# pyprob/pyprob

Hardware: NVIDIA H100
Metric: ic_train_traces_per_sec (higher is better)
Workload: dtype f32

## Files before the change

pyprob_b200/csrc/obs_embed.inc:

```

struct ObsLayout {
  int in_off[PPB_MAX_OBS], out_off[PPB_MAX_OBS];
  int max_depth;
};
inline ObsLayout obs_layout(const ppb_net_desc& D) {
  ObsLayout o;
  int ci = 0, co = 0;
  o.max_depth = 0;
  for (int j = 0; j < D.num_obs; ++j) {
    o.in_off[j] = ci; o.out_off[j] = co;
    ci += D.obs_ff[j].in_dim; co += D.obs_ff[j].out_dim;
    o.max_depth = D.obs_ff[j].num_layers > o.max_depth ? D.obs_ff[j].num_layers : o.max_depth;
  }
  return o;
}

template <class W>
void obs_fp32_plan_fwd(Builder& bl, const ppb_net_desc& D, const float* arena, const float* obs, int B, const W& w,
                       float* obs_emb) {
  const int E = D.obs_dim;
  const ObsLayout o = obs_layout(D);
  for (int l = 0; l < o.max_depth; ++l) {
    bl.begin();
    for (int j = 0; j < D.num_obs; ++j) {
// ... 92 lines not shown

inline obsmlp::Plan obs_plan_of(const ppb_net_desc& D, const Ws* w, const float* obs) {
  obsmlp::Plan P;
  memset(&P, 0, sizeof(P));
  const int E = D.obs_dim;
  const ObsLayout lay = obs_layout(D);
  P.E = E;
  int nf = 0;
  auto add_layer = [&](const ppb_linear_desc& L) -> obsmlp::Layer& {
    obsmlp::Layer& o = P.L[P.n_layers++];
    o.in_dim = L.in_dim; o.out_dim = L.out_dim; o.w_off = L.w_off; o.b_off = L.b_off;
    o.pitch = (L.in_dim & 3) ? L.in_dim : ((L.in_dim & 7) ? L.in_dim : L.in_dim + 4);
    o.sw = nf;
    nf += (L.out_dim * o.pitch + L.out_dim + 3) & ~3;
    o.part = P.part_floats;
    P.part_floats += L.out_dim * L.in_dim + L.out_dim;
    return o;
  };
  std::vector<int> first(D.num_obs);
  for (int j = 0; j < D.num_obs; ++j) {
    const ppb_ff_desc& ff = D.obs_ff[j];
    first[j] = P.n_layers;
    for (int l = 0; l < ff.num_layers; ++l) {
      obsmlp::Layer& o = add_layer(ff.layers[l]);
      o.xoff = P.A; P.A += o.in_dim;
      if (l + 1 < ff.num_layers) { o.dzoff = P.Dz; P.Dz += o.out_dim; }
      o.dxoff = l == 0 ? -1 : P.L[P.n_layers - 2].dzoff;
      o.x = l == 0 ? obs + lay.in_off[j] : (w ? w->obs_act[j][l - 1] : nullptr);
      o.ldx = l == 0 ? D.obs_in_total : ff.layers[l - 1].out_dim;
      if (l + 1 < ff.num_layers) { o.y = w ? w->obs_act[j][l] : nullptr; o.ldy = o.out_dim; }
    }
  }
  const int cat = P.A, dcat = P.Dz;
  P.A += E; P.Dz += E;
  for (int j = 0; j < D.num_obs; ++j) {
    obsmlp::Layer& o = P.L[first[j] + D.obs_ff[j].num_layers - 1];
    o.yoff = cat + lay.out_off[j]; o.dzoff = dcat + lay.out_off[j];
    o.y = w ? w->obs_cat + lay.out_off[j] : nullptr; o.ldy = E;
  }
  for (int j = 0; j < D.num_obs; ++j)
    for (int l = 0; l + 1 < D.obs_ff[j].num_layers; ++l) P.L[first[j] + l].yoff = P.L[first[j] + l + 1].xoff;
  const int nfin = D.obs_final.num_layers;
  for (int l = 0; l < nfin; ++l) {
    const bool last = l == nfin - 1;
    obsmlp::Layer& o = add_layer(D.obs_final.layers[l]);
    if (l == 0) o.xoff = cat;
    o.yoff = P.A; P.A += o.out_dim;
    o.dzoff = P.Dz; P.Dz += o.out_dim;
    o.dxoff = l == 0 ? dcat : P.L[P.n_layers - 2].dzoff;
    o.x = l == 0 ? (w ? w->obs_cat : nullptr) : (w ? w->fin_act[l - 1] : nullptr);
    o.ldx = o.in_dim;
    o.y = w ? (last ? w->obs_emb : w->fin_act[l]) : nullptr; o.ldy = o.out_dim;
    if (l > 0) o.xoff = P.L[P.n_layers - 2].yoff;
  }
  P.w_floats = nf;
  return P;
}
inline bool obs_fused_ok(const ppb_net_desc& D) {
  constexpr int kFuseMaxWidth = obsmlp::W2;
  if (D.obs_dim > kFuseMaxWidth) return false;
  for (int j = 0; j < D.num_obs; ++j)
    for (int l = 0; l < D.obs_ff[j].num_layers; ++l)
      if (D.obs_ff[j].layers[l].in_dim > kFuseMaxWidth || D.obs_ff[j].layers[l].out_dim > kFuseMaxWidth) return false;
  for (int l = 0; l < D.obs_final.num_layers; ++l)
    if (D.obs_final.layers[l].in_dim > kFuseMaxWidth || D.obs_final.layers[l].out_dim > kFuseMaxWidth) return false;
  const obsmlp::Plan P = obs_plan_of(D, nullptr, nullptr);
  return obsmlp::smem_fwd(P) <= obsmlp::kMaxSmem && obsmlp::smem_bwd(P) <= obsmlp::kMaxSmem;
}
int obs_fused_fwd(const ppb_net_desc& D, const float* arena, const float* obs, int B, const Ws& w, cudaStream_t st,
                  const HImg* emb_img = nullptr) {
  int rc = smem_opt_in<obsmlp::k_fwd>(obsmlp::kMaxSmem);
  if (rc) return rc;
  obsmlp::Plan P = obs_plan_of(D, &w, obs);
  if (emb_img) {
    P.emb_k_hi = emb_img->k_hi; P.emb_k_lo = emb_img->k_lo; P.emb_mn_hi = emb_img->mn_hi; P.emb_mn_lo = emb_img->mn_lo;
    P.emb_kb = emb_img->kb;
  }
  const int tpc = (B + PPB_NUM_SMS - 1) / PPB_NUM_SMS;
  PPB_CUDA(ppb_launch(obsmlp::k_fwd, dim3((B + tpc - 1) / tpc), dim3(obsmlp::kThreads), obsmlp::smem_fwd(P), st, 1, 0, P, arena,
                      B, tpc));
  PPB_LAUNCH_CHECK();
  return PPB_OK;
}
int obs_fused_bwd(const ppb_net_desc& D, const float* arena, float* grad, const float* obs, int B, const Ws& w,
                  cudaStream_t st) {
  int rc = smem_opt_in<obsmlp::k_bwd>(obsmlp::kMaxSmem);
  if (rc) return rc;
  const obsmlp::Plan P = obs_plan_of(D, &w, obs);
  constexpr int kMaxCtas = 16 * obsmlp::kCluster;
  int tpc = (B + kMaxCtas - 1) / kMaxCtas;
  tpc = tpc < obsmlp::kMT ? obsmlp::kMT : tpc;
  int ctas = (B + tpc - 1) / tpc;
  ctas = (ctas + obsmlp::kCluster - 1) / obsmlp::kCluster * obsmlp::kCluster;
  PPB_CUDA(ppb_launch(obsmlp::k_bwd, dim3(ctas), dim3(obsmlp::kThreads), obsmlp::smem_bwd(P), st, 1, obsmlp::kCluster, P, arena,
                      (const float*)w.d_obs_emb, grad, B, tpc));
  PPB_LAUNCH_CHECK();
  return PPB_OK;
}

inline bool obs_tc_ok(const ppb_net_desc& D) {
  const ObsLayout o = obs_layout(D);
  for (int j = 0; j < D.num_obs; ++j) {
    const ppb_ff_desc& ff = D.obs_ff[j];
    if (ff.num_layers < 2 || (o.out_off[j] & 31)) return false;
    for (int l = 1; l < ff.num_layers; ++l)
      if (ff.layers[l].in_dim < 32) return false;
  }
  for (int l = 0; l < D.obs_final.num_layers; ++l)
    if (D.obs_final.layers[l].in_dim < 32) return false;
  return true;
}

template <class Add>
void obs_weight_images(ppb_net* net, Add add) {
  const ppb_net_desc& D = net->desc;
  net->obs_form = obs_fused_ok(D) ? ObsForm::fused : obs_tc_ok(D) ? ObsForm::tensor_core : ObsForm::simt;
  if (net->obs_form != ObsForm::tensor_core) return;
  for (int j = 0; j < D.num_obs; ++j)
    for (int l = 1; l < D.obs_ff[j].num_layers; ++l) {
      const ppb_linear_desc& L = D.obs_ff[j].layers[l];
      net->w_obs[j][l] = add(L.w_off, L.out_dim, L.in_dim, L.in_dim);
    }
  for (int l = 0; l < D.obs_final.num_layers; ++l) {
    const ppb_linear_desc& L = D.obs_final.layers[l];
    net->w_fin[l] = add(L.w_off, L.out_dim, L.in_dim, L.in_dim);
  }
}

struct ObsImgs {
  HImg act[PPB_MAX_OBS][PPB_MAX_FF_LAYERS], cat, fin[PPB_MAX_FF_LAYERS];
  HImg g_act[PPB_MAX_OBS][PPB_MAX_FF_LAYERS], g_cat, g_fin[PPB_MAX_FF_LAYERS], g_emb;
  char* begin; int64_t bytes;
};
template <class Img>
void obs_carve_images(const ppb_net* net, int B, Img img, ObsImgs& o) {
  if (net->obs_form != ObsForm::tensor_core) return;
  const ppb_net_desc& D = net->desc;
  for (int j = 0; j < D.num_obs; ++j)
    for (int l = 0; l + 1 < D.obs_ff[j].num_layers; ++l) {
      o.act[j][l] = img(B, D.obs_ff[j].layers[l].out_dim);
      o.g_act[j][l] = img(B, D.obs_ff[j].layers[l].out_dim);
    }
  o.cat = img(B, D.obs_dim);
  o.g_cat = img(B, D.obs_dim);
  for (int l = 0; l + 1 < D.obs_final.num_layers; ++l) {
    o.fin[l] = img(B, D.obs_final.layers[l].out_dim);
    o.g_fin[l] = img(B, D.obs_final.layers[l].out_dim);
  }
  o.g_emb = img(B, D.obs_dim);
}

__global__ void __launch_bounds__(256) k_pack_rows_masked(float* __restrict__ g, const float* __restrict__ y, int rows,
                                                           int cols, int64_t ld, HImg img) {
  ppb_pdl_trigger();
  ppb_pdl_wait();
  tc::pack_tile<tc::Parts::both>(blockIdx.x, (int)img.kb, img.k_hi, img.k_lo, img.mn_hi, img.mn_lo,
                                 [&](int row, int k0, float (&x)[4]) {
#pragma unroll
    for (int j = 0; j < 4; ++j) {
      x[j] = 0.0f;
      if (row < rows && k0 + j < cols) {
        const int64_t o = (int64_t)row * ld + k0 + j;
        x[j] = y[o] > 0.0f ? g[o] : 0.0f;
        g[o] = x[j];
      }
    }
  });
}

struct ObsStep {
  Builder bl;
  std::vector<int> tc_ph;
  int tc_dw = -1;
};

int obs_plan_fwd(ppb_net* net, const float* arena, const ppb_batch* b, const Ws& w, const ObsImgs& im, const HImg& emb_img,
                 TcBuilder& tb, ObsStep& os, cudaStream_t st) {
  const ppb_net_desc& D = net->desc;
// ... 57 lines not shown
  if (net->obs_form != ObsForm::tensor_core) {
    if (!emb_packed) {
      PPB_CUDA(ppb_launch(k_pack_rows, dim3(dim3((B + 127) / 128, 4)), dim3(256), 0, st, 1, 0, w.obs_emb, B, E, E, emb_img));
      PPB_LAUNCH_CHECK();
    }
    return stream_after(net, s_img, st);
  }
  for (int j = 0; j < D.num_obs; ++j) {
    const int od = D.obs_ff[j].layers[0].out_dim;
    PPB_CUDA(ppb_launch(k_pack_rows, dim3(dim3((B + 127) / 128, 4)), dim3(256), 0, st, 1, 0, w.obs_act[j][0], B, od, od, im.act[j][0]));
    PPB_LAUNCH_CHECK();
  }
  rc = stream_after(net, s_img, st); if (rc) return rc;
  for (int ph : os.tc_ph) { rc = run_tc_phase_auto<2>(tb.phases[ph], tdev, precision, st, tb); if (rc) return rc; }
  return PPB_OK;
}

int obs_plan_bwd(ppb_net* net, const float* arena, float* grad, const ppb_batch* b, const Ws& w, const ObsImgs& im,
                 TcBuilder& tb, ObsStep& os, cudaStream_t st) {
  const ppb_net_desc& D = net->desc;
  const int B = b->n_traces;
  const ObsLayout o = obs_layout(D);
  if (net->obs_form == ObsForm::simt) obs_fp32_plan_bwd(os.bl, D, arena, grad, b->obs, B, w);
  if (net->obs_form == ObsForm::tensor_core) {
    os.bl.begin();
    for (int j = 0; j < D.num_obs; ++j) {
      const ppb_linear_desc& L = D.obs_ff[j].layers[0];
      os.bl.add(linear_dw(w.d_obs_act[j][0], L.out_dim, b->obs + o.in_off[j], D.obs_in_total, grad + L.w_off, L.in_dim, B,
                          L.out_dim, L.in_dim));
    }
  }
  int rc = upload_and_get(net, os.bl, w.problems + w.max_problems / 2, w.max_problems / 2, st, 1);
  if (rc) return rc;
  if (net->obs_form != ObsForm::tensor_core) return PPB_OK;
  struct DwSpec { const HImg* gy; int gy_col0; const HImg* x; const ppb_linear_desc* L; };
  std::vector<DwSpec> dws;
  auto add_dx = [&](const ppb_linear_desc& L, const HImg& gy, int gy_col0, const WImg& wi, const HImg& x, float* c,
                    const HImg& gx) {
    tcg::Problem p = TP0();
    p.a = op_k(gy.k_hi, gy.k_lo, (int)gy.kb, 0, gy_col0);
    p.b = wmn(net, wi);
    p.M = B; p.N = L.in_dim; p.K = L.out_dim;
    p.flags = tcg::kMaskImg; p.mask_hi = x.k_hi;
    p.o_k_hi = gx.k_hi; p.o_k_lo = gx.k_lo; p.o_mn_hi = gx.mn_hi; p.o_mn_lo = gx.mn_lo;
    p.o_kb = (int)gx.kb; p.o_row0 = 0; p.o_col0 = 0; p.c = c; p.ldc = L.in_dim;
    tb.add(p);
    dws.push_back({&gy, gy_col0, &x, &L});
  };
  for (int l = D.obs_final.num_layers - 1; l >= 0; --l) {
    const ppb_linear_desc& L = D.obs_final.layers[l];
    os.tc_ph.push_back((int)tb.phases.size());
    tb.begin();
    add_dx(L, (l == D.obs_final.num_layers - 1) ? im.g_emb : im.g_fin[l], 0, net->w_fin[l], l == 0 ? im.cat : im.fin[l - 1],
           l == 0 ? w.d_obs_cat : w.d_fin_act[l - 1], l == 0 ? im.g_cat : im.g_fin[l - 1]);
  }
  for (int l = o.max_depth - 1; l >= 1; --l) {
    os.tc_ph.push_back((int)tb.phases.size());
    tb.begin();
    for (int j = 0; j < D.num_obs; ++j) {
      const ppb_ff_desc& ff = D.obs_ff[j];
      if (l >= ff.num_layers) continue;
      const bool last = l == ff.num_layers - 1;
      add_dx(ff.layers[l], last ? im.g_cat : im.g_act[j][l], last ? o.out_off[j] : 0, net->w_obs[j][l], im.act[j][l - 1],
             w.d_obs_act[j][l - 1], im.g_act[j][l - 1]);
    }
  }
  os.tc_dw = (int)tb.phases.size();
  tb.begin();
  int dw_tiles = 0;
  for (auto& s : dws) dw_tiles += ((s.L->out_dim + 127) / 128) * ((s.L->in_dim + 127) / 128);
  for (auto& s : dws) {
    tcg::Problem p = TP0();
    p.a = op_mn(s.gy->mn_hi, s.gy->mn_lo, (int)s.gy->kb, 0, s.gy_col0);
    p.b = op_mn(s.x->mn_hi, s.x->mn_lo, (int)s.x->kb, 0, 0);
    p.M = s.L->out_dim; p.N = s.L->in_dim; p.K = pad128(B);
    p.c = grad + s.L->w_off; p.ldc = s.L->in_dim;
    p.k_splits = pick_splits(p.M, p.N, p.K, dw_tiles);
    tb.add(p);
  }
  return PPB_OK;
}

int obs_bwd(ppb_net* net, const float* arena, float* grad, const ppb_batch* b, const Ws& w, const ObsImgs& im,
            const TcBuilder& tb, const tcg::Problem* tdev, const ObsStep& os, int precision, cudaStream_t st) {
  const ppb_net_desc& D = net->desc;
  const int B = b->n_traces, E = D.obs_dim;
  const Problem* dev = w.problems + w.max_problems / 2;
  if (net->obs_form == ObsForm::fused) return obs_fused_bwd(D, arena, grad, b->obs, B, w, st);
  if (net->obs_form == ObsForm::simt) return obs_fp32_bwd(os.bl, 0, dev, D, grad, B, w, st);
  PPB_CUDA(ppb_launch(k_pack_rows_masked, dim3(dim3((B + 127) / 128, 4)), dim3(256), 0, st, 1, 0, w.d_obs_emb, w.obs_emb, B, E, E, im.g_emb));
  PPB_LAUNCH_CHECK();
  int rc;
  for (int ph : os.tc_ph) { rc = run_tc_phase_auto<2>(tb.phases[ph], tdev, precision, st, tb); if (rc) return rc; }
  rc = run_tc_phase<1>(tb.phases[os.tc_dw], tdev, precision, st); if (rc) return rc;
  for (int l = 0; l < D.obs_final.num_layers; ++l) {
    const ppb_linear_desc& L = D.obs_final.layers[l];
    const float* dY = (l == D.obs_final.num_layers - 1) ? w.d_obs_emb : w.d_fin_act[l];
    rc = obs_bias_grad(L, dY, L.out_dim, B, grad, st); if (rc) return rc;
  }
  const ObsLayout o = obs_layout(D);
  for (int j = 0; j < D.num_obs; ++j) {
    const ppb_ff_desc& ff = D.obs_ff[j];
    for (int l = 0; l < ff.num_layers; ++l) {
      const ppb_linear_desc& L = ff.layers[l];
      const bool last = l == ff.num_layers - 1;
      const float* dY = last ? w.d_obs_cat + o.out_off[j] : w.d_obs_act[j][l];
      rc = obs_bias_grad(L, dY, last ? E : L.out_dim, B, grad, st); if (rc) return rc;
    }
  }
  return run_phase(os.bl.phases[0], dev, st);
}
```

pyprob_b200/csrc/obs_mlp.cuh:

```cuda
#pragma once
#include "common.cuh"
#include "tc.cuh"
#include "tc_cluster.cuh"

namespace obsmlp {

constexpr int W2 = 96;
constexpr int kThreads = 256;
constexpr int kSlices = 8;
constexpr int kRows = kThreads / kSlices;
constexpr int kMT = 4;
constexpr int kCluster = 8;
constexpr int kMaxLayers = PPB_MAX_OBS * PPB_MAX_FF_LAYERS + PPB_MAX_FF_LAYERS;
constexpr size_t kMaxSmem = 227 * 1024;

struct Layer {
  int in_dim, out_dim;
  int sw, pitch;
  int xoff, yoff;
  int dzoff, dxoff;
  int part;
  int64_t w_off, b_off;
  float* y; int ldy;
  const float* x; int ldx;
};

struct Plan {
  int n_layers;
  int A, Dz;
  int w_floats, part_floats;
  int E;
  Layer L[kMaxLayers];
  float* emb_k_hi; float* emb_k_lo; float* emb_mn_hi; float* emb_mn_lo;
  long long emb_kb;
};

inline size_t smem_fwd(const Plan& p) { return (size_t)(p.w_floats + kMT * p.A) * sizeof(float); }
inline size_t smem_bwd(const Plan& p) { return (size_t)(p.w_floats + p.part_floats + kMT * (p.A + p.Dz)) * sizeof(float); }

__device__ __forceinline__ void cp_async16(float* smem_dst, const float* gmem_src) {
  asm volatile("cp.async.cg.shared.global [%0], [%1], 16;" ::"r"((uint32_t)__cvta_generic_to_shared(smem_dst)), "l"(gmem_src)
               : "memory");
}
__device__ __forceinline__ void cp_async4(float* smem_dst, const float* gmem_src) {
  asm volatile("cp.async.ca.shared.global [%0], [%1], 4;" ::"r"((uint32_t)__cvta_generic_to_shared(smem_dst)), "l"(gmem_src)
               : "memory");
}
__device__ __forceinline__ void cp_async_wait_all() {
  asm volatile("cp.async.commit_group;" ::: "memory");
  asm volatile("cp.async.wait_group 0;" ::: "memory");
}

__device__ __forceinline__ void stage_layer(float* smem, const float* __restrict__ arena, const Layer& L) {
  const int in_dim = L.in_dim, out_dim = L.out_dim, pitch = L.pitch;
  float* dst = smem + L.sw;
  const float* src = arena + L.w_off;
  const float* bsrc = arena + L.b_off;
  if ((in_dim & 3) == 0) {
    const int q = in_dim >> 2, nq = out_dim * q;
    for (int c = threadIdx.x; c < nq; c += kThreads) {
      const int n = c / q, k4 = c - n * q;
      cp_async16(dst + n * pitch + 4 * k4, src + 4 * c);
    }
  } else {
    const int nw = out_dim * in_dim;
    for (int c = threadIdx.x; c < nw; c += kThreads) cp_async4(dst + c, src + c);
  }
  float* bias = dst + out_dim * pitch;
  for (int n = threadIdx.x; n < out_dim; n += kThreads) cp_async4(bias + n, bsrc + n);
}
__device__ __forceinline__ void load_rows(float* dst, int pitch, const float* src, int64_t ld, int tr0, int nt, int width) {
  for (int idx = threadIdx.x; idx < nt * width; idx += kThreads) {
    const int t = idx / width, k = idx - t * width;
    cp_async4(dst + t * pitch + k, src + (int64_t)(tr0 + t) * ld + k);
  }
}

__device__ __forceinline__ float group_sum(float v) {
  v += __shfl_xor_sync(0xffffffffu, v, 4);
  v += __shfl_xor_sync(0xffffffffu, v, 2);
  v += __shfl_xor_sync(0xffffffffu, v, 1);
  return v;
}
__device__ __forceinline__ float pick(const float (&a)[kMT], int i) {
  float r = a[0];
#pragma unroll
  for (int t = 1; t < kMT; ++t) r = i == t ? a[t] : r;
  return r;
}

__device__ __forceinline__ void layer_fwd(const Plan& P, const Layer& L, const float* smem, float* act, int tr0, int nt,
                                          bool last) {
  const int g = threadIdx.x / kSlices, s = threadIdx.x % kSlices;
  const int in_dim = L.in_dim, out_dim = L.out_dim, pitch = L.pitch, A = P.A, ldy = L.ldy;
  const float* w = smem + L.sw;
  const float* bias = w + out_dim * pitch;
  const float* xr = act + L.xoff;
  float* yr = act + L.yoff;
  float* y = L.y;
  float* ek_hi = last ? P.emb_k_hi : nullptr;
  float* ek_lo = P.emb_k_lo;
  float* em_hi = P.emb_mn_hi;
  float* em_lo = P.emb_mn_lo;
  const long long kb = P.emb_kb;
  for (int n = g; n - (g & 3) < out_dim; n += kRows) {
    float acc[kMT];
#pragma unroll
    for (int t = 0; t < kMT; ++t) acc[t] = 0.f;
    const float* wr = w + n * pitch;
    const int kend = n < out_dim ? in_dim : 0;
    for (int k = s; k < kend; k += kSlices) {
      const float wv = wr[k];
#pragma unroll
      for (int t = 0; t < kMT; ++t) acc[t] = fmaf(wv, xr[t * A + k], acc[t]);
    }
#pragma unroll
    for (int t = 0; t < kMT; ++t) acc[t] = group_sum(acc[t]);
    if (s < nt && n < out_dim) {
      const float v = fmaxf(pick(acc, s) + bias[n], 0.f);
      const int tr = tr0 + s;
      yr[s * A + n] = v;
      y[(int64_t)tr * ldy + n] = v;
      if (ek_hi) {
        float hi, lo;
        tc::split_tf32(v, hi, lo);
        const int64_t ok = tc::packed_offset(tr, n, kb);
        ek_hi[ok] = hi;
        if (ek_lo) ek_lo[ok] = lo;
        if (em_hi) {
          const int64_t om = tc::packed_offset_mn(tr, n, kb);
          em_hi[om] = hi;
          if (em_lo) em_lo[om] = lo;
        }
      }
    }
  }
}

__global__ void __launch_bounds__(kThreads) k_fwd(const __grid_constant__ Plan P, const float* __restrict__ arena, int B,
                                                  int traces_per_cta) {
  ppb_pdl_wait();
  ppb_pdl_trigger();
  extern __shared__ __align__(16) float smem[];
  const int n_layers = P.n_layers, A = P.A;
  float* act = smem + P.w_floats;
  for (int i = 0; i < n_layers; ++i) stage_layer(smem, arena, P.L[i]);
  const int t_begin = blockIdx.x * traces_per_cta;
  const int t_end = min(B, t_begin + traces_per_cta);
  for (int c0 = t_begin; c0 < t_end; c0 += kMT) {
    const int nt = min(kMT, t_end - c0);
    for (int i = 0; i < n_layers; ++i) {
      const Layer& L = P.L[i];
      if (L.dxoff < 0) load_rows(act + L.xoff, A, L.x, L.ldx, c0, nt, L.in_dim);
    }
    cp_async_wait_all();
    __syncthreads();
    for (int i = 0; i < n_layers; ++i) {
      layer_fwd(P, P.L[i], smem, act, c0, nt, i == n_layers - 1);
      __syncthreads();
    }
  }
}

__device__ __forceinline__ void layer_dx(const Plan& P, const Layer& L, const float* smem, const float* act, float* dz,
                                         int nt) {
  const int g = threadIdx.x / kSlices, s = threadIdx.x % kSlices;
  const int in_dim = L.in_dim, out_dim = L.out_dim, pitch = L.pitch, A = P.A, Dz = P.Dz;
  const float* w = smem + L.sw;
  const float* dr = dz + L.dzoff;
  const float* xr = act + L.xoff;
  float* dxr = dz + L.dxoff;
  for (int k = g; k - (g & 3) < in_dim; k += kRows) {
    float acc[kMT];
#pragma unroll
    for (int t = 0; t < kMT; ++t) acc[t] = 0.f;
    const int nend = k < in_dim ? out_dim : 0;
    for (int n = s; n < nend; n += kSlices) {
      const float wv = w[n * pitch + k];
#pragma unroll
      for (int t = 0; t < kMT; ++t) acc[t] = fmaf(wv, dr[t * Dz + n], acc[t]);
    }
#pragma unroll
    for (int t = 0; t < kMT; ++t) acc[t] = group_sum(acc[t]);
    if (s < nt && k < in_dim) dxr[s * Dz + k] = xr[s * A + k] > 0.f ? pick(acc, s) : 0.f;
  }
}

__device__ __forceinline__ void layer_partial(const Plan& P, const Layer& L, const float* act, const float* dz, float* part,
                                              int nt) {
  const int in_dim = L.in_dim, out_dim = L.out_dim, A = P.A, Dz = P.Dz;
  const int nw = out_dim * in_dim;
  const float* dr = dz + L.dzoff;
  const float* xr = act + L.xoff;
  float* pr = part + L.part;
  for (int e = threadIdx.x; e < nw + out_dim; e += kThreads) {
    float v = 0.f;
    if (e < nw) {
      const int n = e / in_dim, k = e - n * in_dim;
#pragma unroll
      for (int t = 0; t < kMT; ++t)
        if (t < nt) v = fmaf(dr[t * Dz + n], xr[t * A + k], v);
    } else {
#pragma unroll
      for (int t = 0; t < kMT; ++t)
        if (t < nt) v += dr[t * Dz + e - nw];
    }
    pr[e] += v;
  }
}

__global__ void __launch_bounds__(kThreads) k_bwd(const __grid_constant__ Plan P, const float* __restrict__ arena,
                                                  const float* __restrict__ d_emb, float* __restrict__ grad, int B,
                                                  int traces_per_cta) {
  ppb_pdl_trigger();
  extern __shared__ __align__(16) float smem[];
  const int n_layers = P.n_layers, A = P.A, Dz = P.Dz, E = P.E, part_floats = P.part_floats;
  float* act = smem + P.w_floats;
  float* dz = act + kMT * A;
  float* part = dz + kMT * Dz;
  for (int i = 0; i < n_layers; ++i)
    if (P.L[i].dxoff >= 0) stage_layer(smem, arena, P.L[i]);
  for (int i = threadIdx.x; i < part_floats; i += kThreads) part[i] = 0.f;
  ppb_pdl_wait();
  const int t_begin = blockIdx.x * traces_per_cta;
  const int t_end = min(B, t_begin + traces_per_cta);
  const int zoff = P.L[n_layers - 1].dzoff, eoff = P.L[n_layers - 1].yoff;
  const float* emb = P.L[n_layers - 1].y;
  for (int c0 = t_begin; c0 < t_end; c0 += kMT) {
    const int nt = min(kMT, t_end - c0);
    for (int i = 0; i < n_layers; ++i) {
      const Layer& L = P.L[i];
      load_rows(act + L.xoff, A, L.x, L.ldx, c0, nt, L.in_dim);
    }
    load_rows(act + eoff, A, emb, E, c0, nt, E);
    load_rows(dz + zoff, Dz, d_emb, E, c0, nt, E);
    cp_async_wait_all();
    __syncthreads();
    for (int idx = threadIdx.x; idx < nt * E; idx += kThreads) {
      const int t = idx / E, k = idx - t * E;
      if (!(act[t * A + eoff + k] > 0.f)) dz[t * Dz + zoff + k] = 0.f;
    }
    __syncthreads();
    for (int i = n_layers - 1; i >= 0; --i) {
      if (P.L[i].dxoff < 0) continue;
      layer_dx(P, P.L[i], smem, act, dz, nt);
      __syncthreads();
    }
    for (int i = 0; i < n_layers; ++i) layer_partial(P, P.L[i], act, dz, part, nt);
    __syncthreads();
  }
  cp_async_wait_all();
  tcc::cluster_sync_all();
  const uint32_t rank = tcc::cluster_ctarank();
  const uint32_t part_addr = (uint32_t)__cvta_generic_to_shared(part);
  int li = 0, lpart = P.L[0].part, lnext = n_layers > 1 ? P.L[1].part : part_floats, lnw = P.L[0].out_dim * P.L[0].in_dim;
  int64_t lw = P.L[0].w_off, lb = P.L[0].b_off;
  for (int e = rank * kThreads + threadIdx.x; e < part_floats; e += kCluster * kThreads) {
    float v = 0.f;
#pragma unroll
    for (int r = 0; r < kCluster; ++r) v += tcc::ld_cluster(tcc::map_to_rank(part_addr + 4u * (uint32_t)e, (uint32_t)r));
    while (e >= lnext) {
      ++li;
      const Layer& L = P.L[li];
      lpart = L.part; lnw = L.out_dim * L.in_dim; lw = L.w_off; lb = L.b_off;
      lnext = li + 1 < n_layers ? P.L[li + 1].part : part_floats;
    }
    const int le = e - lpart;
    if (v != 0.f) atomicAdd(grad + (le < lnw ? lw + le : lb + (le - lnw)), v);
  }
  tcc::cluster_sync_all();
}

}
```

pyprob_b200/csrc/net_tc.inc:

```

namespace {

__global__ void __launch_bounds__(256) k_pack_table(const float* __restrict__ arena, const PackEntry* __restrict__ tab,
                                                     int n_entries, float* __restrict__ wimg) {
  int tile = blockIdx.x;
  int lo = 0, hi = n_entries - 1;
  while (lo < hi) {
    int mid = (lo + hi + 1) >> 1;
    if (tab[mid].tile_start <= tile) lo = mid; else hi = mid - 1;
  }
  const PackEntry e = tab[lo];
  const int rt = tile - e.tile_start;
  const float* src = arena + e.src_off;
  tc::pack_tile<tc::Parts::both>(rt, e.kb, wimg + e.k_hi, wimg + e.k_lo, wimg + e.mn_hi, wimg + e.mn_lo,
                                 [&](int row, int k0, float (&x)[4]) {
#pragma unroll
    for (int j = 0; j < 4; ++j) x[j] = (row < e.rows && k0 + j < e.cols) ? __ldg(src + (int64_t)row * e.ld + k0 + j) : 0.0f;
  });
}

__global__ void __launch_bounds__(256) k_pack_rows(const float* __restrict__ src, int rows, int cols, int64_t ld,
                                                    HImg img) {
  ppb_pdl_trigger();
  ppb_pdl_wait();
// ... 502 lines not shown

  if (grad_scale != 1.0f) {
    k_scale<<<ew_grid((int64_t)d.R * net->out_pad), 256, 0, st>>>(w.d_out, (int64_t)d.R * net->out_pad, grad_scale);
    PPB_LAUNCH_CHECK();
    PPB_CUDA(ppb_launch(k_pack_rows, dim3(dim3((d.R + 127) / 128, 4)), dim3(256), 0, st, 1, 0, w.d_out, d.R, net->out_pad, net->out_pad, t.d_out));
    PPB_LAUNCH_CHECK();
  }

  TcBuilder tb;
  const HeadChunks hc = head_chunks(net, b, nullptr, tb);
  std::vector<int> hh_a, hh_b;
  for (int s = 0; s < d.NS; ++s) {
    int r0 = b->step_row0_host[s], np = pad128(b->step_nrows_host[s]);
    for (int q = 0; q < np; q += 32)
      if (b->step_t_host[s] > 0) { hh_a.push_back(r0 + q); hh_b.push_back(b->step_prev_row0_host[s] + q); }
  }
  const int hh_a_off = (int)tb.ints.size();
  tb.ints.insert(tb.ints.end(), hh_a.begin(), hh_a.end());
  const int hh_b_off = (int)tb.ints.size();
  tb.ints.insert(tb.ints.end(), hh_b.begin(), hh_b.end());
  PPB_CHECK_ARG((int64_t)tb.ints.size() <= t.max_ints, "chunk list overflow");

  const int ph_dhid = 0;
  add_head_dhid(tb, net, b, w, t);
  const int ph_hw = (int)tb.phases.size();
  tb.begin();
  for (int s = 0; s < d.NS; ++s) {
    int aid = b->step_addr_host[s];
    const ppb_addr_desc& a = net->addrs[aid];
    tcg::Problem p = TP0();
    p.a = op_k(t.d_hid.k_hi, t.d_hid.k_lo, dhkb, b->step_row0_host[s], 0);
    p.b = wmn(net, net->w1[aid]);
    p.M = pad128(b->step_nrows_host[s]); p.N = H; p.K = a.head_hidden;
    p.c = w.dh + (int64_t)b->step_row0_host[s] * H; p.ldc = H;
    p.o_row0 = b->step_row0_host[s];
    tb.add(p);
  }
  const int ph_headw = (int)tb.phases.size();
  add_head_weight_grads(tb, net, grad, t, hc, t.h, H);
  std::vector<int> ph_rec(d.T, -1);
  {
    int st1 = d.NS;
    for (int tt = d.T - 1; tt >= 1; --tt) {
      int st0 = st1;
      while (st0 > 0 && b->step_t_host[st0 - 1] == tt) --st0;
      ph_rec[tt] = (int)tb.phases.size();
      tb.begin();
      for (int s = st0; s < st1; ++s) {
        tcg::Problem p = TP0();
        p.a = op_k(t.dgates.k_hi, t.dgates.k_lo, gkb, b->step_row0_host[s], 0);
        p.b = wmn(net, net->w_hh);
        p.M = pad128(b->step_nrows_host[s]); p.N = H; p.K = H4;
        p.c = w.dh_rec + (int64_t)b->step_prev_row0_host[s] * H; p.ldc = H;
        tb.add(p);
      }
      {
        gemm::Phase& ph = tb.phases.back();
        int rows = 0;
        for (int i = 0; i < ph.count; ++i) rows += tb.probs[ph.first + i].M;
        const int splits = pick_splits(rows, H, H4);
        ph.tiles = 0;
        for (int i = 0; i < ph.count; ++i) {
          tcg::Problem& p = tb.probs[ph.first + i];
          p.k_splits = splits;
          p.tile_start = ph.tiles;
          ph.tiles += p.tiles_m * p.tiles_n * splits;
        }
      }
      st1 = st0;
    }
  }

  const int ph_lstm_w = (int)tb.phases.size();
  tb.begin();
  if (!hh_a.empty()) {
    tcg::Problem p = TP0();
    p.a = op_mn(t.dgates.mn_hi, t.dgates.mn_lo, gkb, 0, 0, t.ints + hh_a_off);
    p.b = op_mn(t.h.mn_hi, t.h.mn_lo, hkb, 0, 0, t.ints + hh_b_off);
    p.M = H4; p.N = H; p.K = 32 * (int)hh_a.size();
    p.c = grad + D.w_hh_off; p.ldc = H;
    p.k_splits = pick_splits(p.M, p.N, p.K);
    tb.add(p);
  }
  {
    tcg::Problem p = TP0();
    p.a = op_mn(t.dpobs.mn_hi, t.dpobs.mn_lo, gkb, 0, 0);
    p.b = op_mn(t.obs_emb.mn_hi, t.obs_emb.mn_lo, (int)t.obs_emb.kb, 0, 0);
    p.M = H4; p.N = E; p.K = pad128(d.B);
    p.c = grad + D.w_ih_off; p.ldc = I;
    p.k_splits = pick_splits(p.M, p.N, p.K);
    tb.add(p);
    tcg::Problem q = TP0();
    q.a = op_k(t.dpobs.k_hi, t.dpobs.k_lo, gkb, 0, 0);
    q.b = wmn(net, net->w_ihE);
    q.M = d.B; q.N = E; q.K = H4;
    q.c = w.d_obs_emb; q.ldc = E;
    q.k_splits = pick_splits(q.M, q.N, q.K);
    tb.add(q);
  }
  ObsStep os;
  rc = obs_plan_bwd(net, arena, grad, b, w, t.obs, tb, os, st);
  if (rc) return rc;
  PPB_CHECK_ARG((int64_t)tb.probs.size() <= t.max_probs / 2, "tensor-core problem list overflow");
  tcg::Problem* tprobs = t.probs + t.max_probs / 2;
  rc = upload_cached(net, 3, tb.probs.data(), tb.probs.size() * sizeof(tcg::Problem), tprobs, st);
  if (rc) return rc;
  rc = upload_cached(net, 4, tb.ints.data(), tb.ints.size() * sizeof(int), t.ints, st);
  if (rc) return rc;

  cudaStream_t s1 = net->side[0], s2 = net->side[1];
  if (d.T > 1) PPB_CUDA(cudaMemsetAsync(w.dh_rec, 0, (size_t)b->row_off_host[d.T - 1] * H * sizeof(float), st));
  PPB_CUDA(cudaMemsetAsync(w.d_pstep, 0, (size_t)((const char*)(w.d_obs_emb + (int64_t)d.B * E) - (const char*)w.d_pstep), st));
  rc = run_tc_phase_auto<2>(tb.phases[ph_dhid], tprobs, precision, st, tb); if (rc) return rc;
  const bool dpobs_fused = (d.B & 127) == 0 && t.dgates.k_hi != nullptr;
  bool dpobs_packed = false;
  const int cs_cell = (d.T == 1 && dpobs_fused) ? phase_cluster(tb.phases[ph_hw], tb, true) : 1;
  if (cs_cell > 1) {
    CellBwdT1Epi re;
    re.gates = w.gates; re.c = w.c; re.row_trace = b->row_trace; re.dgates = dgates; re.pimg = t.dpobs; re.H = H;
    rc = run_tc_phase_cluster<4>(cs_cell, tb.phases[ph_hw], tprobs, precision, st, re); if (rc) return rc;
    dpobs_packed = true;
  } else {
    rc = run_tc_phase_auto<0>(tb.phases[ph_hw], tprobs, precision, st, tb); if (rc) return rc;
    const HImg gimg = d.T > 1 ? t.dgates : HImg();
    float* const dc = d.T > 1 ? w.dc : nullptr;
    for (int tt = d.T - 1; tt >= 0; --tt) {
      int r0 = b->row_off_host[tt], n = b->row_off_host[tt + 1] - r0;
      if (tt + 1 < d.T) { rc = run_tc_phase<1>(tb.phases[ph_rec[tt + 1]], tprobs, precision, st, profile(tb, ph_rec[tt + 1])); if (rc) return rc; }
      if (tt == 0 && dpobs_fused) {
        PPB_CUDA(ppb_launch(k_cell_bwd<true>, dim3(ew_grid((int64_t)n * H)), dim3(256), 0, st, 1, 0, w.gates, w.c, w.dh, w.dh_rec,
                            dc, dgates, w.d_pobs, b->row_prev, b->row_next, b->row_trace, gimg, r0, n, H, tt, t.dpobs));
        dpobs_packed = true;
      } else {
        PPB_CUDA(ppb_launch(k_cell_bwd<false>, dim3(ew_grid((int64_t)n * H)), dim3(256), 0, st, 1, 0, w.gates, w.c, w.dh, w.dh_rec,
                            dc, dgates, w.d_pobs, b->row_prev, b->row_next, b->row_trace, gimg, r0, n, H, tt, HImg()));
      }
      PPB_LAUNCH_CHECK();
    }
  }
  rc = stream_after(net, st, s1); if (rc) return rc;
  rc = run_tc_phase<1>(tb.phases[ph_headw], tprobs, precision, s1); if (rc) return rc;
  rc = launch_head_bias_grad(net, b, w, grad, s1); if (rc) return rc;
  rc = stream_after(net, st, s2); if (rc) return rc;
  rc = launch_step_inputs_bwd(net, arena, grad, b, w, dgates, s2); if (rc) return rc;
  if (!dpobs_packed) {
    PPB_CUDA(ppb_launch(k_pack_rows, dim3(dim3((d.B + 127) / 128, 64)), dim3(256), 0, st, 1, 0, w.d_pobs, d.B, H4, H4, t.dpobs));
    PPB_LAUNCH_CHECK();
  }
  rc = run_tc_phase<1>(tb.phases[ph_lstm_w], tprobs, precision, st, profile(tb, ph_lstm_w)); if (rc) return rc;
  rc = obs_bwd(net, arena, grad, b, w, t.obs, tb, tprobs, os, precision, st); if (rc) return rc;
  rc = stream_after(net, s1, st); if (rc) return rc;
  return stream_after(net, s2, st);
}

}
```

Baseline: 1.638 million.

## Drop cluster DSMEM reduction in obs MLP backward and strength-reduce index math

Removes the 8-CTA thread-block cluster and its distributed shared-memory reduction of per-CTA weight-gradient partials. Each CTA now atomically adds its own partials straight into global grad. This avoids the cluster syncs and cluster scheduling constraints, at the cost of up to eight times more global atomics onto the same addresses. It also splits the layer_partial loop into separate weight and bias loops and replaces the per-element division with incremental n/k index updates.

```diff
diff --git a/pyprob_b200/csrc/obs_embed.inc b/pyprob_b200/csrc/obs_embed.inc
--- a/pyprob_b200/csrc/obs_embed.inc
+++ b/pyprob_b200/csrc/obs_embed.inc
@@ -203,12 +203,10 @@
   int rc = smem_opt_in<obsmlp::k_bwd>(obsmlp::kMaxSmem);
   if (rc) return rc;
   const obsmlp::Plan P = obs_plan_of(D, &w, obs);
-  constexpr int kMaxCtas = 16 * obsmlp::kCluster;
-  int tpc = (B + kMaxCtas - 1) / kMaxCtas;
+  int tpc = (B + obsmlp::kBwdMaxCtas - 1) / obsmlp::kBwdMaxCtas;
   tpc = tpc < obsmlp::kMT ? obsmlp::kMT : tpc;
-  int ctas = (B + tpc - 1) / tpc;
-  ctas = (ctas + obsmlp::kCluster - 1) / obsmlp::kCluster * obsmlp::kCluster;
-  PPB_CUDA(ppb_launch(obsmlp::k_bwd, dim3(ctas), dim3(obsmlp::kThreads), obsmlp::smem_bwd(P), st, 1, obsmlp::kCluster, P, arena,
+  const int ctas = (B + tpc - 1) / tpc;
+  PPB_CUDA(ppb_launch(obsmlp::k_bwd, dim3(ctas), dim3(obsmlp::kThreads), obsmlp::smem_bwd(P), st, 1, 0, P, arena,
                       (const float*)w.d_obs_emb, grad, B, tpc));
   PPB_LAUNCH_CHECK();
   return PPB_OK;
diff --git a/pyprob_b200/csrc/obs_mlp.cuh b/pyprob_b200/csrc/obs_mlp.cuh
--- a/pyprob_b200/csrc/obs_mlp.cuh
+++ b/pyprob_b200/csrc/obs_mlp.cuh
@@ -1,7 +1,6 @@
 #pragma once
 #include "common.cuh"
 #include "tc.cuh"
-#include "tc_cluster.cuh"
 
 namespace obsmlp {
 
@@ -10,7 +9,7 @@
 constexpr int kSlices = 8;
 constexpr int kRows = kThreads / kSlices;
 constexpr int kMT = 4;
-constexpr int kCluster = 8;
+constexpr int kBwdMaxCtas = 128;
 constexpr int kMaxLayers = PPB_MAX_OBS * PPB_MAX_FF_LAYERS + PPB_MAX_FF_LAYERS;
 constexpr size_t kMaxSmem = 227 * 1024;
 
@@ -190,22 +189,27 @@
                                               int nt) {
   const int in_dim = L.in_dim, out_dim = L.out_dim, A = P.A, Dz = P.Dz;
   const int nw = out_dim * in_dim;
-  const float* dr = dz + L.dzoff;
-  const float* xr = act + L.xoff;
-  float* pr = part + L.part;
-  for (int e = threadIdx.x; e < nw + out_dim; e += kThreads) {
+  const float* __restrict__ dr = dz + L.dzoff;
+  const float* __restrict__ xr = act + L.xoff;
+  float* __restrict__ pr = part + L.part;
+  const int dn = kThreads / in_dim, dk = kThreads - dn * in_dim;
+  int n = threadIdx.x / in_dim, k = threadIdx.x - n * in_dim;
+#pragma unroll 2
+  for (int e = threadIdx.x; e < nw; e += kThreads) {
     float v = 0.f;
-    if (e < nw) {
-      const int n = e / in_dim, k = e - n * in_dim;
-#pragma unroll
-      for (int t = 0; t < kMT; ++t)
-        if (t < nt) v = fmaf(dr[t * Dz + n], xr[t * A + k], v);
-    } else {
-#pragma unroll
-      for (int t = 0; t < kMT; ++t)
-        if (t < nt) v += dr[t * Dz + e - nw];
-    }
+#pragma unroll
+    for (int t = 0; t < kMT; ++t)
+      if (t < nt) v = fmaf(dr[t * Dz + n], xr[t * A + k], v);
     pr[e] += v;
+    n += dn; k += dk;
+    if (k >= in_dim) { k -= in_dim; ++n; }
+  }
+  for (int m = threadIdx.x; m < out_dim; m += kThreads) {
+    float v = 0.f;
+#pragma unroll
+    for (int t = 0; t < kMT; ++t)
+      if (t < nt) v += dr[t * Dz + m];
+    pr[nw + m] += v;
   }
 }
 
@@ -250,15 +254,10 @@
     __syncthreads();
   }
   cp_async_wait_all();
-  tcc::cluster_sync_all();
-  const uint32_t rank = tcc::cluster_ctarank();
-  const uint32_t part_addr = (uint32_t)__cvta_generic_to_shared(part);
   int li = 0, lpart = P.L[0].part, lnext = n_layers > 1 ? P.L[1].part : part_floats, lnw = P.L[0].out_dim * P.L[0].in_dim;
   int64_t lw = P.L[0].w_off, lb = P.L[0].b_off;
-  for (int e = rank * kThreads + threadIdx.x; e < part_floats; e += kCluster * kThreads) {
-    float v = 0.f;
-#pragma unroll
-    for (int r = 0; r < kCluster; ++r) v += tcc::ld_cluster(tcc::map_to_rank(part_addr + 4u * (uint32_t)e, (uint32_t)r));
+  for (int e = threadIdx.x; e < part_floats; e += kThreads) {
+    const float v = part[e];
     while (e >= lnext) {
       ++li;
       const Layer& L = P.L[li];
@@ -268,7 +267,6 @@
     const int le = e - lpart;
     if (v != 0.f) atomicAdd(grad + (le < lnw ? lw + le : lb + (le - lnw)), v);
   }
-  tcc::cluster_sync_all();
-}
-
-}
+}
+
+}
```

New measurement: 1.672 million (median of 6 runs). 1.02x the previous value.

## Form d_obs_emb inside fused observe-embedding backward kernel via cluster reduction

Applied to the files above, without the earlier changes.

When the observe embedding uses the fused form, the separate tensor-core GEMM that computes d_obs_emb from dpobs and w_ihE is dropped. The fused backward kernel now stages slices of w_ih, reads gate gradients (gathering by row when needed) and reduces partial products across the CTA cluster through distributed shared memory. The LSTM weight-gradient phase and its packing are moved to a side stream so they can overlap. layer_partial is also reworked to batch four outputs per thread with incremental index math. The cost is FP32 SIMT arithmetic in place of tensor cores for this product, plus extra cluster syncs and shared-memory pressure.

```diff
diff --git a/pyprob_b200/csrc/net_tc.inc b/pyprob_b200/csrc/net_tc.inc
--- a/pyprob_b200/csrc/net_tc.inc
+++ b/pyprob_b200/csrc/net_tc.inc
@@ -608,6 +608,7 @@
     p.k_splits = pick_splits(p.M, p.N, p.K);
     tb.add(p);
   }
+  const bool obs_forms_demb = net->obs_form == ObsForm::fused;
   {
     tcg::Problem p = TP0();
     p.a = op_mn(t.dpobs.mn_hi, t.dpobs.mn_lo, gkb, 0, 0);
@@ -616,6 +617,8 @@
     p.c = grad + D.w_ih_off; p.ldc = I;
     p.k_splits = pick_splits(p.M, p.N, p.K);
     tb.add(p);
+  }
+  if (!obs_forms_demb) {
     tcg::Problem q = TP0();
     q.a = op_k(t.dpobs.k_hi, t.dpobs.k_lo, gkb, 0, 0);
     q.b = wmn(net, net->w_ihE);
@@ -669,12 +672,20 @@
   rc = launch_head_bias_grad(net, b, w, grad, s1); if (rc) return rc;
   rc = stream_after(net, st, s2); if (rc) return rc;
   rc = launch_step_inputs_bwd(net, arena, grad, b, w, dgates, s2); if (rc) return rc;
+  cudaStream_t s_w = obs_forms_demb ? s2 : st;
   if (!dpobs_packed) {
-    PPB_CUDA(ppb_launch(k_pack_rows, dim3(dim3((d.B + 127) / 128, 64)), dim3(256), 0, st, 1, 0, w.d_pobs, d.B, H4, H4, t.dpobs));
+    PPB_CUDA(ppb_launch(k_pack_rows, dim3(dim3((d.B + 127) / 128, 64)), dim3(256), 0, s_w, 1, 0, w.d_pobs, d.B, H4, H4, t.dpobs));
     PPB_LAUNCH_CHECK();
   }
-  rc = run_tc_phase<1>(tb.phases[ph_lstm_w], tprobs, precision, st, profile(tb, ph_lstm_w)); if (rc) return rc;
-  rc = obs_bwd(net, arena, grad, b, w, t.obs, tb, tprobs, os, precision, st); if (rc) return rc;
+  rc = run_tc_phase<1>(tb.phases[ph_lstm_w], tprobs, precision, s_w, profile(tb, ph_lstm_w)); if (rc) return rc;
+  DembSrc src;
+  src.dp = cs_cell > 1 ? dgates : w.d_pobs;
+  src.ld_dp = H4;
+  const bool by_row = src.dp == dgates && d.R != d.B;
+  src.trace_sub = by_row ? b->trace_sub : nullptr;
+  src.step_row0 = by_row ? b->step_row0 : nullptr;
+  src.row_trace = by_row ? b->row_trace : nullptr;
+  rc = obs_bwd(net, arena, grad, b, w, t.obs, tb, tprobs, os, precision, st, obs_forms_demb ? &src : nullptr); if (rc) return rc;
   rc = stream_after(net, s1, st); if (rc) return rc;
   return stream_after(net, s2, st);
 }
diff --git a/pyprob_b200/csrc/obs_embed.inc b/pyprob_b200/csrc/obs_embed.inc
--- a/pyprob_b200/csrc/obs_embed.inc
+++ b/pyprob_b200/csrc/obs_embed.inc
@@ -198,18 +198,36 @@
   PPB_LAUNCH_CHECK();
   return PPB_OK;
 }
+struct DembSrc {
+  const float* dp; int64_t ld_dp;
+  const int* trace_sub; const int* step_row0; const int* row_trace;
+};
+
 int obs_fused_bwd(const ppb_net_desc& D, const float* arena, float* grad, const float* obs, int B, const Ws& w,
-                  cudaStream_t st) {
+                  cudaStream_t st, const DembSrc* src = nullptr, int64_t ld_wih = 0) {
   int rc = smem_opt_in<obsmlp::k_bwd>(obsmlp::kMaxSmem);
   if (rc) return rc;
-  const obsmlp::Plan P = obs_plan_of(D, &w, obs);
+  obsmlp::Plan P = obs_plan_of(D, &w, obs);
+  size_t smem = obsmlp::smem_bwd(P);
+  if (src) {
+    P.G = 4 * D.lstm_dim;
+    P.wih_off = D.w_ih_off; P.ld_wih = ld_wih;
+    P.wih_vec = (P.E & 3) == 0 && (ld_wih & 3) == 0 && (D.w_ih_off & 3) == 0;
+    P.dp = src->dp; P.ld_dp = src->ld_dp;
+    P.trace_sub = src->trace_sub; P.step_row0 = src->step_row0; P.row_trace = src->row_trace;
+    int kg = P.G / obsmlp::kCluster;
+    while (kg > 4 && obsmlp::smem_emb(P, kg) > obsmlp::kMaxSmem) kg = (kg / 2 + 3) & ~3;
+    PPB_CHECK_ARG(obsmlp::smem_emb(P, kg) <= obsmlp::kMaxSmem, "observe-embedding backward: no room for the d obs_emb chunks");
+    P.kg = kg;
+    smem = std::max(smem, obsmlp::smem_emb(P, kg));
+  }
   constexpr int kMaxCtas = 16 * obsmlp::kCluster;
   int tpc = (B + kMaxCtas - 1) / kMaxCtas;
   tpc = tpc < obsmlp::kMT ? obsmlp::kMT : tpc;
   int ctas = (B + tpc - 1) / tpc;
   ctas = (ctas + obsmlp::kCluster - 1) / obsmlp::kCluster * obsmlp::kCluster;
-  PPB_CUDA(ppb_launch(obsmlp::k_bwd, dim3(ctas), dim3(obsmlp::kThreads), obsmlp::smem_bwd(P), st, 1, obsmlp::kCluster, P, arena,
-                      (const float*)w.d_obs_emb, grad, B, tpc));
+  PPB_CUDA(ppb_launch(obsmlp::k_bwd, dim3(ctas), dim3(obsmlp::kThreads), smem, st, 1, obsmlp::kCluster, P, arena, w.d_obs_emb,
+                      grad, B, tpc));
   PPB_LAUNCH_CHECK();
   return PPB_OK;
 }
@@ -433,11 +451,12 @@
 }
 
 int obs_bwd(ppb_net* net, const float* arena, float* grad, const ppb_batch* b, const Ws& w, const ObsImgs& im,
-            const TcBuilder& tb, const tcg::Problem* tdev, const ObsStep& os, int precision, cudaStream_t st) {
+            const TcBuilder& tb, const tcg::Problem* tdev, const ObsStep& os, int precision, cudaStream_t st,
+            const DembSrc* src = nullptr) {
   const ppb_net_desc& D = net->desc;
   const int B = b->n_traces, E = D.obs_dim;
   const Problem* dev = w.problems + w.max_problems / 2;
-  if (net->obs_form == ObsForm::fused) return obs_fused_bwd(D, arena, grad, b->obs, B, w, st);
+  if (net->obs_form == ObsForm::fused) return obs_fused_bwd(D, arena, grad, b->obs, B, w, st, src, net->I);
   if (net->obs_form == ObsForm::simt) return obs_fp32_bwd(os.bl, 0, dev, D, grad, B, w, st);
   PPB_CUDA(ppb_launch(k_pack_rows_masked, dim3(dim3((B + 127) / 128, 4)), dim3(256), 0, st, 1, 0, w.d_obs_emb, w.obs_emb, B, E, E, im.g_emb));
   PPB_LAUNCH_CHECK();
diff --git a/pyprob_b200/csrc/obs_mlp.cuh b/pyprob_b200/csrc/obs_mlp.cuh
--- a/pyprob_b200/csrc/obs_mlp.cuh
+++ b/pyprob_b200/csrc/obs_mlp.cuh
@@ -33,10 +33,20 @@
   Layer L[kMaxLayers];
   float* emb_k_hi; float* emb_k_lo; float* emb_mn_hi; float* emb_mn_lo;
   long long emb_kb;
+  int G, kg;
+  int64_t wih_off, ld_wih; int wih_vec;
+  const float* dp; int64_t ld_dp;
+  const int* trace_sub; const int* step_row0; const int* row_trace;
 };
 
 inline size_t smem_fwd(const Plan& p) { return (size_t)(p.w_floats + kMT * p.A) * sizeof(float); }
 inline size_t smem_bwd(const Plan& p) { return (size_t)(p.w_floats + p.part_floats + kMT * (p.A + p.Dz)) * sizeof(float); }
+constexpr int kRoundTraces = kCluster * kMT;
+__host__ __device__ inline int emb_wp(int E) { return (E + 3) & ~3; }
+inline size_t smem_emb(const Plan& p, int kg) {
+  const int wp = emb_wp(p.E);
+  return (size_t)(p.w_floats + kg * wp + kRoundTraces * (kg + 4) + kRoundTraces * wp) * sizeof(float);
+}
 
 __device__ __forceinline__ void cp_async16(float* smem_dst, const float* gmem_src) {
   asm volatile("cp.async.cg.shared.global [%0], [%1], 16;" ::"r"((uint32_t)__cvta_generic_to_shared(smem_dst)), "l"(gmem_src)
@@ -188,29 +198,156 @@
 
 __device__ __forceinline__ void layer_partial(const Plan& P, const Layer& L, const float* act, const float* dz, float* part,
                                               int nt) {
+  constexpr int kBatch = 4;
   const int in_dim = L.in_dim, out_dim = L.out_dim, A = P.A, Dz = P.Dz;
   const int nw = out_dim * in_dim;
   const float* dr = dz + L.dzoff;
   const float* xr = act + L.xoff;
   float* pr = part + L.part;
-  for (int e = threadIdx.x; e < nw + out_dim; e += kThreads) {
+  const int dn = kThreads / in_dim, dk = kThreads - dn * in_dim;
+  int n = threadIdx.x / in_dim, k = threadIdx.x - n * in_dim;
+  for (int e = threadIdx.x; e < nw; e += kBatch * kThreads) {
+    float v[kBatch];
+#pragma unroll
+    for (int j = 0; j < kBatch; ++j) {
+      v[j] = 0.f;
+      const bool in = e + j * kThreads < nw;
+#pragma unroll
+      for (int t = 0; t < kMT; ++t) {
+        const bool on = in && t < nt;
+        const float d = on ? dr[t * Dz + n] : 0.f, x = on ? xr[t * A + k] : 0.f;
+        v[j] = fmaf(d, x, v[j]);
+      }
+      n += dn; k += dk;
+      if (k >= in_dim) { k -= in_dim; ++n; }
+    }
+#pragma unroll
+    for (int j = 0; j < kBatch; ++j)
+      if (e + j * kThreads < nw) pr[e + j * kThreads] += v[j];
+  }
+  for (int o = threadIdx.x; o < out_dim; o += kThreads) {
     float v = 0.f;
-    if (e < nw) {
-      const int n = e / in_dim, k = e - n * in_dim;
-#pragma unroll
-      for (int t = 0; t < kMT; ++t)
-        if (t < nt) v = fmaf(dr[t * Dz + n], xr[t * A + k], v);
-    } else {
-#pragma unroll
-      for (int t = 0; t < kMT; ++t)
-        if (t < nt) v += dr[t * Dz + e - nw];
-    }
-    pr[e] += v;
+#pragma unroll
+    for (int t = 0; t < kMT; ++t) v += t < nt ? dr[t * Dz + o] : 0.f;
+    pr[nw + o] += v;
+  }
+}
+
+__device__ __forceinline__ void stage_wih(const Plan& P, const float* __restrict__ arena, float* wsl, int g0, int kg) {
+  const int E = P.E, wp = emb_wp(E);
+  const int64_t ld = P.ld_wih;
+  const float* src = arena + P.wih_off + (int64_t)g0 * ld;
+  if (P.wih_vec) {
+    const int q = E >> 2;
+    for (int c = threadIdx.x; c < kg * q; c += kThreads) {
+      const int g = c / q, k4 = c - g * q;
+      cp_async16(wsl + g * wp + 4 * k4, src + g * ld + 4 * k4);
+    }
+  } else {
+    for (int c = threadIdx.x; c < kg * E; c += kThreads) {
+      const int g = c / E, e = c - g * E;
+      cp_async4(wsl + g * wp + e, src + g * ld + e);
+    }
+  }
+}
+
+__device__ __forceinline__ void form_d_emb(const Plan& P, const float* __restrict__ arena, float* buf, float* d_emb, int B,
+                                           int traces_per_cta) {
+  const int E = P.E, wp = emb_wp(E), KG = P.kg, dpp = KG + 4, gs = P.G / kCluster;
+  float* wsl = buf;
+  float* dps = wsl + KG * wp;
+  float* pb = dps + kRoundTraces * dpp;
+  const uint32_t rank = tcc::cluster_ctarank();
+  const int cbase = (int)(blockIdx.x - rank) * traces_per_cta;
+  const int g_first = (int)rank * gs;
+  const int nch = (gs + KG - 1) / KG, rounds = (traces_per_cta + kMT - 1) / kMT;
+  const int np = (E + 1) >> 1;
+  const float* dp = P.dp;
+  const int64_t ld_dp = P.ld_dp;
+  const int* trace_sub = P.trace_sub; const int* step_row0 = P.step_row0; const int* row_trace = P.row_trace;
+  const uint32_t pb_addr = (uint32_t)__cvta_generic_to_shared(pb);
+  for (int c = 0; c < rounds; ++c) {
+    float acc[2][kMT][2];
+#pragma unroll
+    for (int k = 0; k < 2; ++k)
+#pragma unroll
+      for (int t = 0; t < kMT; ++t) acc[k][t][0] = acc[k][t][1] = 0.f;
+    for (int ch = 0; ch < nch; ++ch) {
+      const int g0 = ch * KG, kg = min(KG, gs - g0);
+      if (c > 0 || ch > 0) {
+        __syncthreads();
+        if (nch > 1) stage_wih(P, arena, wsl, g_first + g0, kg);
+      }
+      const int q4 = kg >> 2;
+      for (int idx = threadIdx.x; idx < kRoundTraces * q4; idx += kThreads) {
+        const int j = idx / q4, k4 = idx - j * q4;
+        const int i = c * kMT + (j % kMT);
+        const int tr = cbase + (j / kMT) * traces_per_cta + i;
+        if (i >= traces_per_cta || tr >= B) continue;
+        int row = tr;
+        if (trace_sub) {
+          const int r0 = __ldg(step_row0 + __ldg(trace_sub + tr));
+          row = r0 + tr - __ldg(row_trace + r0);
+        }
+        cp_async16(dps + j * dpp + 4 * k4, dp + (int64_t)row * ld_dp + g_first + g0 + 4 * k4);
+      }
+      cp_async_wait_all();
+      __syncthreads();
+#pragma unroll
+      for (int k = 0; k < 2; ++k) {
+        const int it = threadIdx.x + k * kThreads;
+        if (it >= kRoundTraces / kMT * np) continue;
+        const int q = it / np, p = it - q * np;
+        const float* dr = dps + q * kMT * dpp;
+        const float* wr = wsl + 2 * p;
+#pragma unroll 2
+        for (int g = 0; g < kg; g += 4) {
+          float d[kMT][4];
+#pragma unroll
+          for (int t = 0; t < kMT; ++t) {
+            const float4 v = *reinterpret_cast<const float4*>(dr + t * dpp + g);
+            d[t][0] = v.x; d[t][1] = v.y; d[t][2] = v.z; d[t][3] = v.w;
+          }
+#pragma unroll
+          for (int u = 0; u < 4; ++u) {
+            const float2 w = *reinterpret_cast<const float2*>(wr + (g + u) * wp);
+#pragma unroll
+            for (int t = 0; t < kMT; ++t) {
+              acc[k][t][0] = fmaf(d[t][u], w.x, acc[k][t][0]);
+              acc[k][t][1] = fmaf(d[t][u], w.y, acc[k][t][1]);
+            }
+          }
+        }
+      }
+    }
+#pragma unroll
+    for (int k = 0; k < 2; ++k) {
+      const int it = threadIdx.x + k * kThreads;
+      if (it >= kRoundTraces / kMT * np) continue;
+      const int q = it / np, p = it - q * np;
+#pragma unroll
+      for (int t = 0; t < kMT; ++t) {
+        pb[(q * kMT + t) * wp + 2 * p] = acc[k][t][0];
+        pb[(q * kMT + t) * wp + 2 * p + 1] = acc[k][t][1];
+      }
+    }
+    tcc::cluster_sync_all();
+    for (int idx = threadIdx.x; idx < kMT * E; idx += kThreads) {
+      const int t = idx / E, e = idx - t * E;
+      const int i = c * kMT + t, tr = cbase + (int)rank * traces_per_cta + i;
+      if (i >= traces_per_cta || tr >= B) continue;
+      const uint32_t a = pb_addr + 4u * (uint32_t)(((int)rank * kMT + t) * wp + e);
+      float v = 0.f;
+#pragma unroll
+      for (int r = 0; r < kCluster; ++r) v += tcc::ld_cluster(tcc::map_to_rank(a, (uint32_t)r));
+      d_emb[(int64_t)tr * E + e] = v;
+    }
+    tcc::cluster_sync_all();
   }
 }
 
 __global__ void __launch_bounds__(kThreads) k_bwd(const __grid_constant__ Plan P, const float* __restrict__ arena,
-                                                  const float* __restrict__ d_emb, float* __restrict__ grad, int B,
+                                                  float* __restrict__ d_emb, float* __restrict__ grad, int B,
                                                   int traces_per_cta) {
   ppb_pdl_trigger();
   extern __shared__ __align__(16) float smem[];
@@ -220,8 +357,15 @@
   float* part = dz + kMT * Dz;
   for (int i = 0; i < n_layers; ++i)
     if (P.L[i].dxoff >= 0) stage_layer(smem, arena, P.L[i]);
-  for (int i = threadIdx.x; i < part_floats; i += kThreads) part[i] = 0.f;
+  const bool form = P.G > 0;
+  if (form) stage_wih(P, arena, act, (int)tcc::cluster_ctarank() * (P.G / kCluster), min(P.kg, P.G / kCluster));
+  else for (int i = threadIdx.x; i < part_floats; i += kThreads) part[i] = 0.f;
   ppb_pdl_wait();
+  if (form) {
+    form_d_emb(P, arena, act, d_emb, B, traces_per_cta);
+    for (int i = threadIdx.x; i < part_floats; i += kThreads) part[i] = 0.f;
+    __syncthreads();
+  }
   const int t_begin = blockIdx.x * traces_per_cta;
   const int t_end = min(B, t_begin + traces_per_cta);
   const int zoff = P.L[n_layers - 1].dzoff, eoff = P.L[n_layers - 1].yoff;
```

Result: faster. 1.635 million before, 1.736 million after, median of 6 (+6.2%).
